# bbuchfink/diamond

Hardware: AMD Instinct MI355X
Metric: GCUPS + aligned queries/s, blastp --fast, 10000 queries vs 1000000-seq DB (seed stage + banded SW extension) (higher is better)
Workload: dtype int16

## Files before the change

### diamond_amd/csrc/api.hip

```cpp
#include <hip/hip_runtime.h>
#include <algorithm>
#include <atomic>
#include <chrono>
#include <time.h>
#include <cstdio>
#include <cstdlib>
#include <cstring>
#include <mutex>
#include <thread>
#include <numeric>
#include <unordered_map>
#include <string>
#include <vector>
#include "../../include/diamond_hip.h"
#include "swipe_core.h"
#include "swipe16_core.h"
#include "host_pool.h"
#include "swipe_kernels.h"
#include "ctx.h"
#include "score_matrices.h"

using namespace dmnd;

static thread_local std::string g_last_error;

int dmnd::fail(int code, const std::string& msg)
{
	g_last_error = msg;
	return code;
}

namespace {
std::mutex g_sync_mutex;
std::unordered_map<hipStream_t, hipEvent_t> g_sync_events;
}

static int sync_spin_us()
{
	return tuning().sync_spin_us;
}

hipError_t dmnd::wait_event(hipEvent_t ev, double* hint_us)
{
	if (spin_sync()) return hipEventSynchronize(ev);
	const int spin_us = sync_spin_us();
	auto t0 = std::chrono::steady_clock::now();
	const auto t_wait = t0;
	double fine_until_us = 0.0;
	auto finish = [&](hipError_t e) {
		if (hint_us) *hint_us = e == hipSuccess ? std::chrono::duration<double, std::micro>(std::chrono::steady_clock::now() - t_wait).count() : 0.0;
		return e;
	};
	if (hint_us && *hint_us > 2.0 * spin_us) {
		const hipError_t q = hipEventQuery(ev);
		if (q != hipErrorNotReady) return finish(q);
		const long ns = (long)(std::min(*hint_us, 50000.0) * 750.0);
		timespec ts{ 0, ns };
		nanosleep(&ts, nullptr);
		t0 = std::chrono::steady_clock::now();
		fine_until_us = 2.0 * std::min(*hint_us, 50000.0);
	}
	long sleep_ns = 20000;
	for (;;) {
		const hipError_t q = hipEventQuery(ev);
		if (q == hipSuccess) return finish(hipSuccess);
		if (q != hipErrorNotReady) return finish(q);
		if (std::chrono::duration_cast<std::chrono::microseconds>(std::chrono::steady_clock::now() - t0).count() < spin_us) continue;
		timespec ts{ 0, sleep_ns };
		nanosleep(&ts, nullptr);
		if (sleep_ns < 200000) sleep_ns += sleep_ns / 2;
		if (fine_until_us > 0.0 && sleep_ns > 50000 && std::chrono::duration<double, std::micro>(std::chrono::steady_clock::now() - t_wait).count() < fine_until_us) sleep_ns = 50000;
	}
}

hipError_t dmnd::sync_stream(hipStream_t s, double* hint_us)
{
	if (spin_sync()) return hipStreamSynchronize(s);
	hipEvent_t ev = nullptr;
	{
		std::lock_guard<std::mutex> g(g_sync_mutex);
		auto it = g_sync_events.find(s);
		if (it != g_sync_events.end()) ev = it->second;
		else {
			const hipError_t e = hipEventCreateWithFlags(&ev, hipEventBlockingSync | hipEventDisableTiming);
			if (e != hipSuccess) return e;
			g_sync_events[s] = ev;
		}
	}
	const hipError_t e = hipEventRecord(ev, s);
	if (e != hipSuccess) return e;
	return wait_event(ev, hint_us);
}

void dmnd::forget_stream(hipStream_t s)
{
	hipEvent_t ev = nullptr;
	{
		std::lock_guard<std::mutex> g(g_sync_mutex);
		auto it = g_sync_events.find(s);
// ... 421 lines not shown
	HIP_TRY(hipSetDevice(c->device));
	c->cbs_len = len;
	if (len == 0)
		return DMND_OK;
	c->cbs_generation = ~(uint64_t)0;
	if (int rc = c->cbs.ensure((size_t)len + 256)) return rc;
	HIP_TRY(hipMemcpyAsync(c->cbs.p, cbs, (size_t)len, hipMemcpyHostToDevice, c->stream));
	HIP_TRY(sync_stream(c->stream));
	return DMND_OK;
}

extern "C" int32_t dmnd_banded_cols(int32_t qlen, int32_t tlen, int32_t d_begin, int32_t d_end)
{
	const int32_t pos = std::max(d_end - 1, 0) - (d_end - 1);
	const int32_t j1 = std::min(qlen - 1 - d_begin, tlen - 1) + 1;
	return j1 - pos;
}

extern "C" double dmnd_evalue(const dmnd_ctx* c, int32_t raw_score, uint32_t query_len, uint32_t subject_len)
{
	return c ? c->evaluer.evalue(raw_score, query_len, subject_len) : 0.0;
}

extern "C" double dmnd_evalue_p(const dmnd_params* p, int32_t raw_score, uint32_t query_len, uint32_t subject_len)
{
	if (!p) return 0.0;
	Evaluer e;
	e.init(*p);
	return e.evalue(raw_score, query_len, subject_len);
}

extern "C" int dmnd_evalue_batch(const dmnd_params* p, const int32_t* raw_score, const int32_t* query_len, const int32_t* subject_len,
	int64_t n, double* out)
{
	if (!p || !raw_score || !query_len || !subject_len || !out || n < 0) return fail(DMND_E_ARG, "dmnd_evalue_batch: bad argument");
	Evaluer e;
	e.init(*p);
	for (int64_t i = 0; i < n; ++i)
		out[i] = e.evalue(raw_score[i], (unsigned)query_len[i], (unsigned)subject_len[i]);
	return DMND_OK;
}

extern "C" double dmnd_bitscore_p(const dmnd_params* p, double raw_score)
{
	if (!p) return 0.0;
	Evaluer e;
	e.init(*p);
	return e.bitscore(raw_score);
}

extern "C" double dmnd_bitscore(const dmnd_ctx* c, double raw_score)
{
	return c ? c->evaluer.bitscore(raw_score) : 0.0;
}

extern "C" int dmnd_last_kernel_ms(const dmnd_ctx* c, double* swipe_ms, double* traceback_ms)
{
	if (!c) return fail(DMND_E_ARG, "ctx is NULL");
	if (swipe_ms) *swipe_ms = c->swipe_ms;
	if (traceback_ms) *traceback_ms = c->traceback_ms;
	return DMND_OK;
}

namespace {

struct Bases {
	const int8_t* q; int64_t q_len;
	const int8_t* t; int64_t t_len;
	const int8_t* cbs; int64_t cbs_len;
	const int8_t* matrices = nullptr; int64_t n_matrices = 0;
};

enum { ADJ_CLASS = 1 << 20 };
struct Slot { int32_t item; int32_t P; int64_t steps; };
inline int band_p(const Slot& s) { return s.P & (ADJ_CLASS - 1); }
inline bool own_matrix(const Slot& s) { return (s.P & ADJ_CLASS) != 0; }

bool force_swipe32()
{
	static const bool v = [] { const char* e = std::getenv("DMND_SWIPE32"); return e && e[0] == '1'; }();
	return v;
}

}

int64_t dmnd::sweep_rows_min_items()
{
	if (force_swipe32()) return INT64_MAX;
	const char* e = std::getenv("DMND_SWEEP_ROWS");
	if (e && e[0] == '0') return INT64_MAX;
	if (e && e[0] == '1') return 0;
	return tuning().sweep_rows_min_items;
}

namespace {

inline int sweep_class(int band, int64_t steps, bool own, int kmode, bool rows)
{
	if (rows && !own && kmode <= K_TRACE && steps <= 2 * (int64_t)SW16_MAX_PAIRS) return band_class_rows(band);
	return band_class(band);
}

struct SweepLaunch { int64_t s0, s1; bool k16; int64_t pair_off; };

void plan_sweeps(const std::vector<Slot>& slots, int kmode, bool force32, std::vector<SweepLaunch>& launches, std::vector<int32_t>& pairs)
{
	const int64_t n = (int64_t)slots.size();
	launches.clear(); pairs.clear();
	for (int64_t s0 = 0; s0 < n;) {
		int64_t s1 = s0, max_steps = 0;
		while (s1 < n && slots[(size_t)s1].P == slots[(size_t)s0].P) { max_steps = std::max(max_steps, slots[(size_t)s1].steps); ++s1; }
		const bool k16 = !force32 && !force_swipe32() && kmode <= K_TRACE && !own_matrix(slots[(size_t)s0]) && sw16_class(slots[(size_t)s0].P) && max_steps <= 2 * (int64_t)SW16_MAX_PAIRS;
		launches.push_back(SweepLaunch{ s0, s1, k16, (int64_t)pairs.size() });
		if (k16) {
			const int64_t per = class_items_per_wave16(slots[(size_t)s0].P);
			for (int64_t s = s0; s < (s1 - s0 + per - 1) / per * per + s0; ++s)
				pairs.push_back(s < s1 ? slots[(size_t)s].item : -1);
		}
		s0 = s1;
	}
}

int issue_sweeps(dmnd_ctx* work, const Bases& b, const dmnd_dp_target* d_items, const std::vector<Slot>& slots, const std::vector<SweepLaunch>& launches,
	const int32_t* order_dev, const int64_t* trace_off_slot_dev, const int32_t* pairs_dev, const int64_t* trace_off_item_dev, uint8_t* trace_dev, int kmode)
{
	const bool trace = kmode == K_TRACE;
	for (const SweepLaunch& l : launches) {
		const int P = band_p(slots[(size_t)l.s0]);
		if (l.k16) {
			Swipe16Args a;
			a.qblock = b.q; a.tblock = b.t; a.cbs = b.cbs; a.matrix = work->matrix.as<int8_t>();
			a.items = d_items;
			a.pairs = pairs_dev + l.pair_off;
			a.trace_off = trace ? trace_off_item_dev : nullptr;
			a.trace = trace ? trace_dev : nullptr;
			a.ends = work->ends.as<SwipeEnd>();
			a.n_pairs = (l.s1 - l.s0 + class_items_per_wave16(P) - 1) / class_items_per_wave16(P);
			a.gap_open = work->params.gap_open; a.gap_extend = work->params.gap_extend;
			a.score_only = kmode == K_SCORE;
			HIP_TRY(launch_banded_swipe16(P, trace, a, work->stream));
		}
		else {
			SwipeArgs a;
			a.qblock = b.q; a.tblock = b.t; a.cbs = b.cbs; a.matrix = work->matrix.as<int8_t>(); a.matrices = b.matrices;
			a.items = d_items;
			a.order = order_dev + l.s0;
			a.trace_off = trace ? trace_off_slot_dev + l.s0 : nullptr;
			a.trace = trace ? trace_dev : nullptr;
			a.ends = work->ends.as<SwipeEnd>();
			a.n = l.s1 - l.s0;
			a.gap_open = work->params.gap_open; a.gap_extend = work->params.gap_extend;
			HIP_TRY(launch_banded_swipe(P, kmode, a, work->stream));
		}
	}
	return DMND_OK;
}

int launch_sweeps(dmnd_ctx* work, const Bases& b, const dmnd_dp_target* d_items, int64_t n_items_total, const std::vector<Slot>& slots,
	const int32_t* order_dev, const int64_t* trace_off_slot_dev, const std::vector<int64_t>* trace_off_slot, uint8_t* trace_dev, int kmode, bool force32)
{
	const int64_t n = (int64_t)slots.size();
	const bool trace = kmode == K_TRACE;
	std::vector<SweepLaunch> launches;
	std::vector<int32_t>& pairs = work->h_pairs;
	plan_sweeps(slots, kmode, force32, launches, pairs);
	if (!pairs.empty()) {
		if (int rc = work->pairs.ensure(pairs.size() * sizeof(int32_t))) return rc;
		HIP_TRY(hipMemcpyAsync(work->pairs.p, pairs.data(), pairs.size() * sizeof(int32_t), hipMemcpyHostToDevice, work->stream));
		if (trace) {
			std::vector<int64_t>& by_item = work->h_trace_off_item;
			by_item.assign((size_t)n_items_total, 0);
			for (int64_t s = 0; s < n; ++s) by_item[(size_t)slots[(size_t)s].item] = (*trace_off_slot)[(size_t)s];
			if (int rc = work->trace_off_item.ensure(by_item.size() * sizeof(int64_t))) return rc;
			HIP_TRY(hipMemcpyAsync(work->trace_off_item.p, by_item.data(), by_item.size() * sizeof(int64_t), hipMemcpyHostToDevice, work->stream));
		}
	}
	return issue_sweeps(work, b, d_items, slots, launches, order_dev, trace_off_slot_dev, work->pairs.as<int32_t>(), work->trace_off_item.as<int64_t>(), trace_dev, kmode);
}

void order_slots(std::vector<Slot>& v, std::vector<Slot>& tmp, std::vector<uint32_t>& count)
{
	if (v.size() < 2048) {
		std::sort(v.begin(), v.end(), [](const Slot& x, const Slot& y) { return x.P < y.P || (x.P == y.P && x.steps > y.steps); });
		return;
	}
	const int NB = 1024;
	count.assign((size_t)32 * NB + 1, 0);
	auto cls = [](const Slot& x) { return class_index(band_p(x)) + (own_matrix(x) ? 16 : 0); };
	auto bucket = [&](const Slot& x) { return (size_t)cls(x) * NB + (size_t)(NB - 1 - std::min<int64_t>(x.steps >> 4, NB - 1)); };
	for (const Slot& x : v) ++count[bucket(x) + 1];
	for (size_t i = 1; i < count.size(); ++i) count[i] += count[i - 1];
	tmp.resize(v.size());
	for (const Slot& x : v) tmp[count[bucket(x)]++] = x;
	v.swap(tmp);
}

int run_chunk(dmnd_ctx* c, const Bases& b, const dmnd_dp_target* items, int64_t n_items_total, const dmnd_dp_target* d_items, const std::vector<Slot>& slots,
	int kmode, dmnd_hsp* out, std::vector<uint8_t>* chunk_transcripts, std::vector<int64_t>* chunk_tr_off, bool force32 = false)
{
	const int64_t n = (int64_t)slots.size();
	if (n == 0) return DMND_OK;
	const bool trace = kmode == K_TRACE;
	std::vector<int32_t> order(n), p_of(n);
	std::vector<int64_t> trace_off(n + 1, 0), tr_off(n + 1, 0);
	for (int64_t s = 0; s < n; ++s) {
		order[s] = slots[s].item;
		p_of[s] = band_p(slots[s]);
		if (trace) {
			const dmnd_dp_target& it = items[slots[s].item];
			const Geom g = make_geom(it.query_len, it.target_len, it.d_begin, it.d_end);
			trace_off[s + 1] = trace_off[s] + trace_bytes(g, band_p(slots[s]));
// ... 159 lines not shown
		HIP_TRY(hipMemcpyAsync(c->items.p, rev.data(), m * sizeof(dmnd_dp_target), hipMemcpyHostToDevice, c->stream));
		const double ms_fwd = c->swipe_ms;
		if (int rc = run_chunk(c, b, rev.data(), m, c->items.as<dmnd_dp_target>(), rslots, K_STATS_BWD_REV, out, nullptr, nullptr)) return rc;
		(void)ms_fwd;
		HIP_TRY(copy_now(c->stream, ends.data(), c->ends.p, m * sizeof(SwipeEnd), hipMemcpyDeviceToHost));
		for (int64_t k = 0; k < m; ++k) {
			dmnd_hsp& h = out[src[k]];
			h.score = ends[k].score;
			h.q_begin = rev[k].query_len - (ends[k].end_i + 1);
			h.s_begin = rev[k].target_len - (ends[k].end_j + 1);
			h.mismatches = ends[k].stat_a;
			h.gap_openings = ends[k].stat_b;
			h.gaps = h.length - h.identities - h.mismatches;
		}
		return DMND_OK;
	}

	hsps.resize((size_t)n);
	int64_t used = 0;
	for (int64_t c0 = 0; c0 < n;) {
		int64_t c1 = c0;
		size_t bytes = 0;
		while (c1 < n) {
			const dmnd_dp_target& it = items[c1];
			const Geom g = make_geom(it.query_len, it.target_len, it.d_begin, it.d_end);
			const size_t need = (size_t)trace_bytes(g, band_p(slots[c1]));
			if (c1 > c0 && bytes + need > c->trace_arena_max) break;
			bytes += need;
			++c1;
		}
		std::vector<Slot> chunk(slots.begin() + c0, slots.begin() + c1);
		order_slots(chunk);
		std::vector<uint8_t> tr;
		std::vector<int64_t> tr_off;
		lap(0);
		if (int rc = run_chunk(c, b, items, n, c->items.as<dmnd_dp_target>(), chunk, K_TRACE, out, transcript ? &tr : nullptr, transcript ? &tr_off : nullptr)) return rc;
		lap(1);
		HIP_TRY(copy_now(c->stream, hsps.data() + c0, c->hsps.as<dmnd_hsp>() + c0, (size_t)(c1 - c0) * sizeof(dmnd_hsp), hipMemcpyDeviceToHost));
		std::vector<Slot> again;
		std::vector<uint8_t> tr2;
		std::vector<int64_t> tr_off2;
		for (const Slot& x : chunk) if (hsps[(size_t)x.item].transcript_len < 0) again.push_back(for_32_bits(x));
		if (!again.empty()) {
			std::sort(again.begin(), again.end(), by_class);
			if (int rc = run_chunk(c, b, items, n, c->items.as<dmnd_dp_target>(), again, K_TRACE, out, transcript ? &tr2 : nullptr, transcript ? &tr_off2 : nullptr, true)) return rc;
			for (const Slot& x : again)
				HIP_TRY(copy_now(c->stream, &hsps[(size_t)x.item], c->hsps.as<dmnd_hsp>() + x.item, sizeof(dmnd_hsp), hipMemcpyDeviceToHost));
		}
		if (!transcript) {
			for (int64_t i = c0; i < c1; ++i) { out[i] = hsps[i]; out[i].transcript_off = -1; }
			c0 = c1;
			continue;
		}
		std::vector<int64_t> slot_of((size_t)(c1 - c0)), slot2_of((size_t)(c1 - c0), -1);
		for (size_t s = 0; s < chunk.size(); ++s) slot_of[(size_t)(chunk[s].item - c0)] = (int64_t)s;
		for (size_t s = 0; s < again.size(); ++s) slot2_of[(size_t)(again[s].item - c0)] = (int64_t)s;
		for (int64_t i = c0; i < c1; ++i) {
			dmnd_hsp h = hsps[i];
			const int64_t s2 = slot2_of[(size_t)(i - c0)], s = slot_of[(size_t)(i - c0)];
			const uint8_t* src = s2 >= 0 ? tr2.data() + tr_off2[(size_t)s2] : tr.data() + tr_off[(size_t)s];
			const int64_t len = h.transcript_len + 1;
			if (used + len > transcript_cap)
				return fail(DMND_E_CAP, "dmnd_banded_swipe: transcript arena too small");
			std::memcpy(transcript + used, src, (size_t)len);
			h.transcript_off = used;
			used += len;
			out[i] = h;
		}
		c0 = c1;
	}
	if (transcript_used) *transcript_used = used;
	lap(2);
	return DMND_OK;
}

}

int dmnd_sweep_classes(dmnd_ctx* work, const dmnd_ctx* c, const dmnd_dp_target* d_items, const uint32_t* class_count, const uint32_t* class_max_steps, int n_classes,
	const int32_t* order_dev, const int64_t* off_slot_dev, const int32_t* pairs_dev, const int64_t* off_item_dev, uint8_t* trace_dev, SwipeEnd* ends_dev)
{
	if (!c || !work) return fail(DMND_E_ARG, "ctx is NULL");
	const int8_t* cbs = c->cbs_len > 0 ? c->cbs.as<int8_t>() : nullptr;
	int64_t s0 = 0, pair0 = 0;
	for (int k = 0; k < n_classes; ++k) {
		const int64_t count = class_count[k];
		if (count == 0) continue;
		const bool own = k >= 16;
		const int P = class_of_index(own ? k - 16 : k);
		const int64_t per = class_items_per_wave16(P), waves = (count + per - 1) / per;
		const bool k16 = !own && !force_swipe32() && sw16_class(P) && (int64_t)class_max_steps[k] <= 2 * (int64_t)SW16_MAX_PAIRS;
		if (row_class(P) && !k16) return fail(DMND_E_ARG, "dmnd_sweep_classes: a row class outside the 16-bit kernels");
		if (k16) {
			Swipe16Args a;
			a.qblock = c->block[DMND_QUERY].as<int8_t>(); a.tblock = c->block[DMND_TARGET].as<int8_t>(); a.cbs = cbs; a.matrix = c->matrix.as<int8_t>();
			a.items = d_items; a.pairs = pairs_dev + pair0; a.trace_off = trace_dev ? off_item_dev : nullptr; a.trace = trace_dev; a.ends = ends_dev;
			a.n_pairs = waves;
			a.gap_open = c->params.gap_open; a.gap_extend = c->params.gap_extend;
			a.score_only = trace_dev == nullptr;
			HIP_TRY(launch_banded_swipe16(P, trace_dev != nullptr, a, work->stream));
		}
		else {
			SwipeArgs a;
			a.qblock = c->block[DMND_QUERY].as<int8_t>(); a.tblock = c->block[DMND_TARGET].as<int8_t>(); a.cbs = cbs; a.matrix = c->matrix.as<int8_t>(); a.matrices = own ? work->adj_matrices.as<int8_t>() : nullptr;
			a.items = d_items; a.order = order_dev + s0; a.trace_off = trace_dev ? off_slot_dev + s0 : nullptr; a.trace = trace_dev; a.ends = ends_dev;
			a.n = count;
			a.gap_open = c->params.gap_open; a.gap_extend = c->params.gap_extend;
			HIP_TRY(launch_banded_swipe(P, trace_dev ? K_TRACE : K_SCORE, a, work->stream));
		}
		s0 += count; pair0 += waves * per;
	}
	return DMND_OK;
}

int dmnd_swipe_shared(dmnd_ctx* work, const dmnd_ctx* c, const dmnd_dp_target* items, int64_t n, int mode, uint32_t hsp_values,
	dmnd_hsp* out, uint8_t* transcript, int64_t transcript_cap, int64_t* transcript_used)
{
	if (!c || !work) return fail(DMND_E_ARG, "ctx is NULL");
	const Bases b{ c->block[DMND_QUERY].as<int8_t>(), c->block_len[DMND_QUERY], c->block[DMND_TARGET].as<int8_t>(), c->block_len[DMND_TARGET],
		c->cbs_len > 0 ? c->cbs.as<int8_t>() : nullptr, c->cbs_len, work->adj_matrices.as<int8_t>(), work->n_adj_matrices };
	if (work != c) {
		work->matrix.p = c->matrix.p; work->matrix.cap = c->matrix.cap; work->matrix.own = false;
		work->params = c->params; work->evaluer = c->evaluer;
	}
	return swipe_impl(work, b, items, n, mode, hsp_values, out, transcript, transcript_cap, transcript_used);
}

int dmnd_swipe_targets(dmnd_ctx* work, const dmnd_ctx* c, const int8_t* t, int64_t t_len, const dmnd_dp_target* items, int64_t n, int mode, uint32_t hsp_values,
	dmnd_hsp* out, uint8_t* transcript, int64_t transcript_cap, int64_t* transcript_used)
{
	if (!c || !work || !t) return fail(DMND_E_ARG, "ctx is NULL");
	const Bases b{ c->block[DMND_QUERY].as<int8_t>(), c->block_len[DMND_QUERY], t, t_len, c->cbs_len > 0 ? c->cbs.as<int8_t>() : nullptr, c->cbs_len,
		work->adj_matrices.as<int8_t>(), work->n_adj_matrices };
	if (work != c) {
		work->matrix.p = c->matrix.p; work->matrix.cap = c->matrix.cap; work->matrix.own = false;
		work->params = c->params; work->evaluer = c->evaluer;
	}
	return swipe_impl(work, b, items, n, mode, hsp_values, out, transcript, transcript_cap, transcript_used);
}

int dmnd_swipe_keep(dmnd_ctx* work, const dmnd_ctx* c, const dmnd_dp_target* items, int64_t n, int arena, dmnd_hsp* out, KeptTrace& kt)
{
	kt.arena = arena; kt.kept = false;
	if (!c || !work) return fail(DMND_E_ARG, "ctx is NULL");
	if (n == 0) return DMND_OK;
	const Bases b{ c->block[DMND_QUERY].as<int8_t>(), c->block_len[DMND_QUERY], c->block[DMND_TARGET].as<int8_t>(), c->block_len[DMND_TARGET],
		c->cbs_len > 0 ? c->cbs.as<int8_t>() : nullptr, c->cbs_len, work->adj_matrices.as<int8_t>(), work->n_adj_matrices };
	auto wall = [] { return std::chrono::duration<double, std::milli>(std::chrono::steady_clock::now().time_since_epoch()).count(); };
	const double t0 = wall();
	int64_t total = 0;
	bool usable = arena >= 0 && arena < 16 && n <= 0x7fffffff, in_range = true;
	const bool rows = n >= sweep_rows_min_items();
	static thread_local std::vector<Slot> slots, sort_tmp;
	static thread_local std::vector<uint32_t> sort_count;
	static thread_local std::vector<int64_t> rows_of;
	slots.resize((size_t)n); rows_of.resize((size_t)n);
	for (int64_t i = 0; i < n && usable; ++i) {
		const dmnd_dp_target& it = items[i];
		const int band = it.d_end - it.d_begin;
		if (band <= 0 || it.query_len <= 0 || it.target_len <= 0 || band_class(band) > 32) { usable = false; break; }
		in_range &= !(it.query_off < 0 || it.target_off < 0 || it.query_off + it.query_len > b.q_len || it.target_off + it.target_len > b.t_len
			|| (it.cbs_off >= 0 && (!b.cbs || it.cbs_off + it.query_len > b.cbs_len)) || (it.cbs_off <= -2 && (own_matrix_number(it.cbs_off) >= b.n_matrices || (own_matrix_biased(it.cbs_off) && (!b.cbs || it.query_off + it.query_len > b.cbs_len)))));
		const Geom g = make_geom(it.query_len, it.target_len, it.d_begin, it.d_end);
		const int P = sweep_class(band, n_steps(g), it.cbs_off <= -2, K_TRACE, rows);
		slots[(size_t)i] = Slot{ (int32_t)i, P | (it.cbs_off <= -2 ? (int)ADJ_CLASS : 0), n_steps(g) };
		rows_of[(size_t)i] = trace_bytes(g, P);
		total += rows_of[(size_t)i];
	}
	if (!usable || (size_t)total > work->trace_arena_max)
		return dmnd_swipe_shared(work, c, items, n, DMND_SWIPE_SCORE, 0, out, nullptr, 0, nullptr);
// ... 262 lines not shown
```

### diamond_amd/csrc/swipe16_kernels.hip

```cpp
#include <hip/hip_runtime.h>
#include <stdint.h>
#include <type_traits>
#include <utility>
#include "swipe16_core.h"
#include "swipe_kernels.h"

namespace dmnd {

__device__ __forceinline__ uint32_t shr1_z(uint32_t v) { return (uint32_t)__builtin_amdgcn_update_dpp(0, (int)v, 0x138, 0xf, 0xf, true); }
__device__ __forceinline__ uint32_t shl1_z(uint32_t v) { return (uint32_t)__builtin_amdgcn_update_dpp(0, (int)v, 0x130, 0xf, 0xf, true); }
__device__ __forceinline__ uint32_t shr1_in(uint32_t edge, uint32_t v) { return (uint32_t)__builtin_amdgcn_update_dpp((int)edge, (int)v, 0x138, 0xf, 0xf, false); }
__device__ __forceinline__ uint32_t shl1_in(uint32_t edge, uint32_t v) { return (uint32_t)__builtin_amdgcn_update_dpp((int)edge, (int)v, 0x130, 0xf, 0xf, false); }

__device__ __forceinline__ uint32_t rshr1_z(uint32_t v) { return (uint32_t)__builtin_amdgcn_update_dpp(0, (int)v, 0x111, 0xf, 0xf, true); }
__device__ __forceinline__ uint32_t rshl1_z(uint32_t v) { return (uint32_t)__builtin_amdgcn_update_dpp(0, (int)v, 0x101, 0xf, 0xf, true); }
__device__ __forceinline__ uint32_t rshr1_in(uint32_t edge, uint32_t v) { return (uint32_t)__builtin_amdgcn_update_dpp((int)edge, (int)v, 0x111, 0xf, 0xf, false); }
__device__ __forceinline__ uint32_t rshl1_in(uint32_t edge, uint32_t v) { return (uint32_t)__builtin_amdgcn_update_dpp((int)edge, (int)v, 0x101, 0xf, 0xf, false); }

__device__ __forceinline__ int rfl(int x) { return __builtin_amdgcn_readfirstlane(x); }
__device__ __forceinline__ int64_t rfl64(int64_t x)
{
	const uint32_t lo = (uint32_t)rfl((int)(uint32_t)x), hi = (uint32_t)rfl((int)(uint32_t)((uint64_t)x >> 32));
	return (int64_t)(((uint64_t)hi << 32) | lo);
}

struct Item16 {
	Geom g;
	SeqView v;
	int pairs;
};

__device__ __forceinline__ Item16 load_item(const dmnd_dp_target* items, int idx, const int8_t* qblock, const int8_t* tblock, const int8_t* cbs)
{
	const dmnd_dp_target it = items[idx];
	Item16 r;
	r.g = make_geom(rfl(it.query_len), rfl(it.target_len), rfl(it.d_begin), rfl(it.d_end));
	const int64_t c = rfl64(it.cbs_off);
	r.v = SeqView{ qblock + rfl64(it.query_off), tblock + rfl64(it.target_off), c >= 0 ? cbs + c : nullptr, nullptr };
	r.pairs = sw16_pairs(r.g);
	return r;
}

__device__ __forceinline__ Item16 load_item_row(const dmnd_dp_target* items, int idx, const int8_t* qblock, const int8_t* tblock, const int8_t* cbs)
{
	const dmnd_dp_target it = items[idx];
	Item16 r;
	r.g = make_geom(it.query_len, it.target_len, it.d_begin, it.d_end);
	r.v = SeqView{ qblock + it.query_off, tblock + it.target_off, it.cbs_off >= 0 ? cbs + it.cbs_off : nullptr, nullptr };
	r.pairs = sw16_pairs(r.g);
	return r;
}

template<int... R, typename F>
__device__ __forceinline__ void unrolled(std::integer_sequence<int, R...>, F&& f) { (f(std::integral_constant<int, R>()), ...); }

enum { EDGE_CHUNK = 256 };

template<int P, bool TRACE, bool COORDS = true>
__global__ __launch_bounds__(WAVES_PER_BLOCK * 64)
void banded_swipe16_kernel(const int8_t* __restrict__ qblock, const int8_t* __restrict__ tblock, const int8_t* __restrict__ cbs,
	const int8_t* __restrict__ matrix, const dmnd_dp_target* __restrict__ items, const int32_t* __restrict__ pairs,
	const int64_t* __restrict__ trace_off, uint8_t* __restrict__ trace, SwipeEnd* __restrict__ ends, int64_t n_pairs, int gap_open, int gap_extend)
{
	__shared__ uint16_t table[32 * 32];
	__shared__ uint4 edges[WAVES_PER_BLOCK][EDGE_CHUNK];
	for (int x = threadIdx.x; x < 32 * 32; x += blockDim.x)
		table[x] = sw16_table_entry(matrix, x);
	__syncthreads();

	const int lane = threadIdx.x & 63, wave = rfl((int)(threadIdx.x >> 6));
	const int64_t slot = (int64_t)blockIdx.x * WAVES_PER_BLOCK + wave;
	if (slot >= n_pairs)
		return;
	const int idxA = rfl(pairs[2 * slot]), idxB_raw = rfl(pairs[2 * slot + 1]);
	const bool hasB = idxB_raw >= 0;
	const int idxB = hasB ? idxB_raw : idxA;
	const Item16 A = load_item(items, idxA, qblock, tblock, cbs), B = load_item(items, idxB, qblock, tblock, cbs);
	const pk16 go = pk_both(gap_open + gap_extend), ge = pk_both(gap_extend);
	const int nA = A.pairs, nB = hasB ? B.pairs : 0;

	Lane16<P> st;
	lane16_init(st, A.g, A.v, B.g, B.v, lane);
	constexpr int G = Sw16Group<P>::G;
	uint8_t *recA = nullptr, *recB = nullptr;
	if (TRACE) {
		recA = trace + rfl64(trace_off[idxA]) + lane * 16;
		recB = trace + rfl64(trace_off[idxB]) + lane * 16;
	}
	uint4* const my_edges = edges[wave];

	pk16 S0[P], S1[P];
	lane16_scores(st, table, S0, S1);
	Edge16 e = sw16_edge(A.g, A.v, B.g, B.v, P, 0);
	Trace16Group<P> acc;

	auto pair_step = [&](auto r, int t, int tc) {
		constexpr int R = decltype(r)::value;
		const uint4 nx = my_edges[t - tc];
		lane16_advance(st, shl1_in(e.qq, st.QQ[1]), shl1_in(e.cc, st.CC[1]), shr1_in(e.tt, st.TT[P - 1]));
		pk16 N0[P], N1[P];
		lane16_scores(st, table, N0, N1);
		const uint32_t revt = 0xffffu - (uint32_t)t;
		pk16 tb0[P], tb1[P];
		lane16_step<P, TRACE, 0, COORDS>(st, S0, shr1_z(st.F[2 * P - 1]), go, ge, revt, tb0);
		lane16_step<P, TRACE, 1, COORDS>(st, S1, shl1_z(st.E[0]), go, ge, revt, tb1);
		if (TRACE) acc.template put<R>(tb0, tb1);
#pragma unroll
		for (int p = 0; p < P; ++p) { S0[p] = N0[p]; S1[p] = N1[p]; }
		e.qq = nx.x; e.tt = nx.y; e.cc = nx.z;
		if (R % 2 == 1) __builtin_amdgcn_sched_barrier(0);
	};
	const int nMax = nA > nB ? nA : nB, T = (nMax + G - 1) / G * G;
	for (int tc = 0; tc < T; tc += EDGE_CHUNK) {
		__builtin_amdgcn_wave_barrier();
#pragma unroll
		for (int r = lane; r < EDGE_CHUNK; r += 64) {
			const Edge16 x = sw16_edge(A.g, A.v, B.g, B.v, P, tc + 1 + r);
			my_edges[r] = make_uint4(x.qq, x.tt, x.cc, 0u);
		}
		__builtin_amdgcn_fence(__ATOMIC_RELEASE, "wavefront");
		__builtin_amdgcn_wave_barrier();
		__builtin_amdgcn_fence(__ATOMIC_ACQUIRE, "wavefront");
		const int te = tc + EDGE_CHUNK < T ? tc + EDGE_CHUNK : T;
		for (int t = tc; t < te; t += G) {
			unrolled(std::make_integer_sequence<int, G>(), [&](auto r) { pair_step(r, t + decltype(r)::value, tc); });
			if (TRACE) {
				if (t < nA) *reinterpret_cast<uint4*>(recA) = make_uint4(acc.a[0], acc.a[1], acc.a[2], acc.a[3]);
				if (t < nB) *reinterpret_cast<uint4*>(recB) = make_uint4(acc.b[0], acc.b[1], acc.b[2], acc.b[3]);
				recA += 1024; recB += 1024;
			}
		}
	}

#pragma unroll
	for (int item = 0; item < 2; ++item) {
		if (item == 1 && !hasB) break;
		int bs, bi, bj;
		lane16_finish<P, COORDS>(st, item ? B.g : A.g, item == 1, lane, bs, bi, bj);
#pragma unroll
		for (int off = 32; off >= 1; off >>= 1) {
			const int os = __shfl_xor(bs, off), oi = __shfl_xor(bi, off), oj = __shfl_xor(bj, off);
			if (better_end(os, oj, oi, bs, bj, bi)) { bs = os; bi = oi; bj = oj; }
		}
		if (lane == 0) {
			SwipeEnd x;
			x.score = bs; x.end_i = bi; x.end_j = bj; x.stat_a = 0; x.stat_b = 0;
			x.pad[0] = bs >= SW16_MAX_SCORE ? 1 : 0;
			x.pad[1] = x.pad[2] = 0;
			ends[item ? idxB : idxA] = x;
		}
	}
}

enum { ROW_EDGE_CHUNK = 60 };

template<int P, bool TRACE, bool COORDS = true>
__global__ __launch_bounds__(WAVES_PER_BLOCK * 64)
void banded_swipe16_rows_kernel(const int8_t* __restrict__ qblock, const int8_t* __restrict__ tblock, const int8_t* __restrict__ cbs,
	const int8_t* __restrict__ matrix, const dmnd_dp_target* __restrict__ items, const int32_t* __restrict__ pairs,
	const int64_t* __restrict__ trace_off, uint8_t* __restrict__ trace, SwipeEnd* __restrict__ ends, int64_t n_waves, int gap_open, int gap_extend)
{
	__shared__ uint16_t table[32 * 32];
	__shared__ uint4 edges[WAVES_PER_BLOCK][4][ROW_EDGE_CHUNK + 1];
	for (int x = threadIdx.x; x < 32 * 32; x += blockDim.x)
		table[x] = sw16_table_entry(matrix, x);
	__syncthreads();

	const int lane = threadIdx.x & 63, wave = rfl((int)(threadIdx.x >> 6)), row = lane >> 4, rl = lane & 15;
	const int64_t slot = (int64_t)blockIdx.x * WAVES_PER_BLOCK + wave;
	if (slot >= n_waves)
		return;
	const int idx0 = rfl(pairs[8 * slot]);
	const int idxA_raw = pairs[8 * slot + 2 * row], idxB_raw = pairs[8 * slot + 2 * row + 1];
	const bool hasA = idxA_raw >= 0, hasB = idxB_raw >= 0;
	const int idxA = hasA ? idxA_raw : idx0, idxB = hasB ? idxB_raw : idxA;
	auto again = [](int idx) { asm volatile("" : "+v"(idx)); return idx; };
	const pk16 go = pk_both(gap_open + gap_extend), ge = pk_both(gap_extend);
	int nA, nB;
	Lane16<P> st;
	pk16 S0[P], S1[P];
	Edge16 e;
	{
		const Item16 A = load_item_row(items, idxA, qblock, tblock, cbs), B = load_item_row(items, idxB, qblock, tblock, cbs);
		nA = hasA ? A.pairs : 0; nB = hasB ? B.pairs : 0;
		lane16_init(st, A.g, A.v, B.g, B.v, rl);
		lane16_scores(st, table, S0, S1);
		e = sw16_edge(A.g, A.v, B.g, B.v, P, 0, 15);
	}
	constexpr int G = Sw16Group<P>::G;
	uint8_t *recA = nullptr, *recB = nullptr;
	if (TRACE) {
		recA = trace + trace_off[idxA] + rl * 16;
		recB = trace + trace_off[idxB] + rl * 16;
	}
	uint4* const my_edges = edges[wave][row];
	Trace16Group<P> acc;

	auto pair_step = [&](auto r, int t, int tc) {
		constexpr int R = decltype(r)::value;
		const uint4 nx = my_edges[t - tc];
		lane16_advance(st, rshl1_in(e.qq, st.QQ[1]), rshl1_in(e.cc, st.CC[1]), rshr1_in(e.tt, st.TT[P - 1]));
		pk16 N0[P], N1[P];
		lane16_scores(st, table, N0, N1);
		const uint32_t revt = 0xffffu - (uint32_t)t;
		pk16 tb0[P], tb1[P];
		lane16_step<P, TRACE, 0, COORDS>(st, S0, rshr1_z(st.F[2 * P - 1]), go, ge, revt, tb0);
		lane16_step<P, TRACE, 1, COORDS>(st, S1, rshl1_z(st.E[0]), go, ge, revt, tb1);
		if (TRACE) acc.template put<R>(tb0, tb1);
#pragma unroll
		for (int p = 0; p < P; ++p) { S0[p] = N0[p]; S1[p] = N1[p]; }
		e.qq = nx.x; e.tt = nx.y; e.cc = nx.z;
		__builtin_amdgcn_sched_barrier(0);
	};
	int nMax = nA > nB ? nA : nB;
	nMax = max(max(__builtin_amdgcn_readlane(nMax, 0), __builtin_amdgcn_readlane(nMax, 16)), max(__builtin_amdgcn_readlane(nMax, 32), __builtin_amdgcn_readlane(nMax, 48)));
	const int T = (nMax + G - 1) / G * G;
	for (int tc = 0; tc < T; tc += ROW_EDGE_CHUNK) {
		__builtin_amdgcn_wave_barrier();
		{
			const Item16 A = load_item_row(items, again(idxA), qblock, tblock, cbs), B = load_item_row(items, again(idxB), qblock, tblock, cbs);
			for (int r = rl; r < ROW_EDGE_CHUNK; r += 16) {
				const Edge16 x = sw16_edge(A.g, A.v, B.g, B.v, P, tc + 1 + r, 15);
				my_edges[r] = make_uint4(x.qq, x.tt, x.cc, 0u);
			}
		}
		__builtin_amdgcn_fence(__ATOMIC_RELEASE, "wavefront");
		__builtin_amdgcn_wave_barrier();
		__builtin_amdgcn_fence(__ATOMIC_ACQUIRE, "wavefront");
		const int te = tc + ROW_EDGE_CHUNK < T ? tc + ROW_EDGE_CHUNK : T;
		for (int t = tc; t < te; t += G) {
			unrolled(std::make_integer_sequence<int, G>(), [&](auto r) { pair_step(r, t + decltype(r)::value, tc); });
			if (TRACE) {
				if (t < nA) *reinterpret_cast<uint4*>(recA) = make_uint4(acc.a[0], acc.a[1], acc.a[2], acc.a[3]);
				if (t < nB) *reinterpret_cast<uint4*>(recB) = make_uint4(acc.b[0], acc.b[1], acc.b[2], acc.b[3]);
				recA += 256; recB += 256;
			}
		}
	}

#pragma unroll
	for (int item = 0; item < 2; ++item) {
		const dmnd_dp_target it = items[again(item ? idxB : idxA)];
		const Geom g = make_geom(it.query_len, it.target_len, it.d_begin, it.d_end);
		int bs, bi, bj;
		lane16_finish<P, COORDS>(st, g, item == 1, rl, bs, bi, bj);
#pragma unroll
		for (int off = 8; off >= 1; off >>= 1) {
			const int os = __shfl_xor(bs, off), oi = __shfl_xor(bi, off), oj = __shfl_xor(bj, off);
			if (better_end(os, oj, oi, bs, bj, bi)) { bs = os; bi = oi; bj = oj; }
		}
		if (rl == 0 && (item ? hasB : hasA)) {
			SwipeEnd x;
			x.score = bs; x.end_i = bi; x.end_j = bj; x.stat_a = 0; x.stat_b = 0;
			x.pad[0] = bs >= SW16_MAX_SCORE ? 1 : 0;
			x.pad[1] = x.pad[2] = 0;
			ends[item ? idxB : idxA] = x;
		}
	}
}

template<int P>
static hipError_t launch16_rows(bool trace, const Swipe16Args& a, hipStream_t stream)
{
	const unsigned blocks = (unsigned)((a.n_pairs + WAVES_PER_BLOCK - 1) / WAVES_PER_BLOCK);
	if (blocks == 0)
		return hipSuccess;
	const dim3 grid(blocks), block(WAVES_PER_BLOCK * 64);
	if (trace) hipLaunchKernelGGL((banded_swipe16_rows_kernel<P, true>), grid, block, 0, stream, a.qblock, a.tblock, a.cbs, a.matrix, a.items, a.pairs, a.trace_off, a.trace, a.ends, a.n_pairs, a.gap_open, a.gap_extend);
	else if (a.score_only) hipLaunchKernelGGL((banded_swipe16_rows_kernel<P, false, false>), grid, block, 0, stream, a.qblock, a.tblock, a.cbs, a.matrix, a.items, a.pairs, a.trace_off, a.trace, a.ends, a.n_pairs, a.gap_open, a.gap_extend);
	else hipLaunchKernelGGL((banded_swipe16_rows_kernel<P, false>), grid, block, 0, stream, a.qblock, a.tblock, a.cbs, a.matrix, a.items, a.pairs, a.trace_off, a.trace, a.ends, a.n_pairs, a.gap_open, a.gap_extend);
	return hipGetLastError();
}

template<int P>
static hipError_t launch16_p(bool trace, const Swipe16Args& a, hipStream_t stream)
{
	const unsigned blocks = (unsigned)((a.n_pairs + WAVES_PER_BLOCK - 1) / WAVES_PER_BLOCK);
	if (blocks == 0)
		return hipSuccess;
	const dim3 grid(blocks), block(WAVES_PER_BLOCK * 64);
	if (trace) hipLaunchKernelGGL((banded_swipe16_kernel<P, true>), grid, block, 0, stream, a.qblock, a.tblock, a.cbs, a.matrix, a.items, a.pairs, a.trace_off, a.trace, a.ends, a.n_pairs, a.gap_open, a.gap_extend);
	else if (a.score_only) hipLaunchKernelGGL((banded_swipe16_kernel<P, false, false>), grid, block, 0, stream, a.qblock, a.tblock, a.cbs, a.matrix, a.items, a.pairs, a.trace_off, a.trace, a.ends, a.n_pairs, a.gap_open, a.gap_extend);
	else hipLaunchKernelGGL((banded_swipe16_kernel<P, false>), grid, block, 0, stream, a.qblock, a.tblock, a.cbs, a.matrix, a.items, a.pairs, a.trace_off, a.trace, a.ends, a.n_pairs, a.gap_open, a.gap_extend);
	return hipGetLastError();
}

hipError_t launch_banded_swipe16(int P, bool trace, const Swipe16Args& a, hipStream_t stream)
{
	switch (P) {
	case 1: return launch16_p<1>(trace, a, stream);
	case 2: return launch16_p<2>(trace, a, stream);
	case 4: return launch16_p<4>(trace, a, stream);
	case 3: return launch16_rows<3>(trace, a, stream);
	case 5: return launch16_rows<5>(trace, a, stream);
	default: return hipErrorInvalidValue;
	}
}

}

namespace { __global__ void touch_swipe16_kernel() {} }
extern "C" hipError_t dmnd_touch_swipe16(hipStream_t st) { hipLaunchKernelGGL(touch_swipe16_kernel, dim3(1), dim3(64), 0, st); return hipGetLastError(); }
```

### diamond_amd/csrc/swipe_kernels.h

```cpp
#pragma once
#include <hip/hip_runtime.h>
#include <stdint.h>
#include "../../include/diamond_hip.h"

namespace dmnd {

enum { WAVES_PER_BLOCK = 4 };

struct SwipeEnd {
	int32_t score, end_i, end_j, stat_a, stat_b, pad[3];
};

__host__ __device__ inline int64_t own_matrix_number(int64_t cbs_off) { return (-2 - cbs_off) & (DMND_CBS_MATRIX_WITH_BIAS - 1); }
__host__ __device__ inline bool own_matrix_biased(int64_t cbs_off) { return cbs_off <= -2 && ((-2 - cbs_off) & DMND_CBS_MATRIX_WITH_BIAS) != 0; }

enum { K_SCORE = 0, K_COORDS = 1, K_TRACE = 2, K_STATS_FWD = 3, K_STATS_BWD_REV = 4 };

struct SwipeArgs {
	const int8_t* qblock;
	const int8_t* tblock;
	const int8_t* cbs;
	const int8_t* matrix;
	const int8_t* matrices;
	const dmnd_dp_target* items;
	const int32_t* order;
	const int64_t* trace_off;
	uint8_t* trace;
	SwipeEnd* ends;
	int64_t n;
	int32_t gap_open, gap_extend;
};

struct TracebackArgs {
	const int8_t* qblock;
	const int8_t* tblock;
	const int8_t* cbs;
	const int8_t* matrix;
	const int8_t* matrices;
	const dmnd_dp_target* items;
	const int32_t* order;
	const int32_t* p_of_slot;
	const int64_t* trace_off;
	const int64_t* transcript_off;
	const uint8_t* trace;
	uint8_t* transcript;
	const SwipeEnd* ends;
	dmnd_hsp* hsps;
	int32_t* status;
	int64_t n;
	int32_t gap_open, gap_extend;
	int32_t transcript_from_first = 0;
};

struct Swipe16Args {
	const int8_t* qblock;
	const int8_t* tblock;
	const int8_t* cbs;
	const int8_t* matrix;
	const dmnd_dp_target* items;
	const int32_t* pairs;
	const int64_t* trace_off;
	uint8_t* trace;
	SwipeEnd* ends;
	int64_t n_pairs;
	int32_t gap_open, gap_extend;
	bool score_only = false;
};

hipError_t launch_banded_swipe(int P, int mode, const SwipeArgs& a, hipStream_t stream);
hipError_t launch_banded_swipe16(int P, bool trace, const Swipe16Args& a, hipStream_t stream);
hipError_t launch_traceback(const TracebackArgs& a, hipStream_t stream);

}
```

### diamond_amd/csrc/tuning.h

```cpp
#pragma once
#include <algorithm>
#include <cstdlib>

namespace dmnd {

struct Tuning {
	bool spin_sync = false;
	int sync_spin_us = 150;
	int pool_spins = 600;
	int extend_team = 8;
	int extend_split = 1;
	int extend_runners = 1;
	int extend_sub_threads = 0;
	int sweep_rows_min_items = 1 << 17;
	int extend_resweep_below_pct = 40;
	bool no_stream_priority = false;
	int seed_slots_x8 = 0;
	int seed_readback_bytes = 1 << 20;
	int seed_slices_budget_mb = 3072;
	long long seed_slices_min_letters = 1 << 20;
	long long seed_slices_max_joined = 1 << 20;
	int seed_sort_cap = 1 << 16;
};

inline const Tuning& tuning()
{
	static const Tuning t = [] {
		Tuning x;
		auto num = [](const char* name, int fallback) { const char* e = std::getenv(name); return e ? std::atoi(e) : fallback; };
		{ const char* e = std::getenv("DMND_SPIN_SYNC"); x.spin_sync = e && e[0] == '1'; }
		x.sync_spin_us = std::max(0, num("DMND_SYNC_SPIN_US", x.sync_spin_us));
		x.pool_spins = std::max(0, num("DMND_POOL_SPINS", x.pool_spins));
		x.extend_team = std::max(1, num("DMND_EXTEND_TEAM", x.extend_team));
		x.extend_split = std::max(1, std::min(64, num("DMND_EXTEND_SPLIT", x.extend_split)));
		x.extend_runners = std::max(1, num("DMND_EXTEND_RUNNERS", x.extend_runners));
		x.extend_sub_threads = std::max(0, num("DMND_EXTEND_SUB_THREADS", x.extend_sub_threads));
		x.sweep_rows_min_items = std::max(0, num("DMND_SWEEP_ROWS_MIN", x.sweep_rows_min_items));
		x.extend_resweep_below_pct = std::max(0, std::min(100, num("DMND_EXTEND_RESWEEP_BELOW_PCT", x.extend_resweep_below_pct)));
		x.no_stream_priority = std::getenv("DMND_NO_STREAM_PRIORITY") != nullptr;
		if (std::getenv("DMND_SEED_SLOTS_X8")) x.seed_slots_x8 = std::min(64, std::max(8, num("DMND_SEED_SLOTS_X8", 0)));
		return x;
	}();
	return t;
}

}
```

Before: 253.5.

## Fuse 16-bit banded sweep classes into a single multi-class kernel launch

```diff
diff --git a/diamond_amd/csrc/api.hip b/diamond_amd/csrc/api.hip
--- a/diamond_amd/csrc/api.hip
+++ b/diamond_amd/csrc/api.hip
@@ -15,6 +15,7 @@
 #include "../../include/diamond_hip.h"
 #include "swipe_core.h"
 #include "swipe16_core.h"
+#include "swipe16_fused.h"
 #include "host_pool.h"
 #include "swipe_kernels.h"
 #include "ctx.h"
@@ -602,6 +603,13 @@
 	return v;
 }
 
+bool sweep_fused(int n_classes, bool with_rows, int64_t n_items)
+{
+	const char* e = std::getenv("DMND_SWEEP_FUSED");
+	if (n_classes < 2 || (e && e[0] == '0')) return false;
+	return (e && e[0] == '1') || with_rows || n_items <= tuning().sweep_fused_waves_max_items;
+}
+
 }
 
 int64_t dmnd::sweep_rows_min_items()
@@ -645,8 +653,31 @@
 	const int32_t* order_dev, const int64_t* trace_off_slot_dev, const int32_t* pairs_dev, const int64_t* trace_off_item_dev, uint8_t* trace_dev, int kmode)
 {
 	const bool trace = kmode == K_TRACE;
+	bool fused[FUSED_CLASSES] = { false, false, false, false };
+	{
+		int64_t f_waves[FUSED_CLASSES] = { 0, 0, 0, 0 }, f_pair0[FUSED_CLASSES] = { 0, 0, 0, 0 }, f_items = 0;
+		int n_fused = 0;
+		for (const SweepLaunch& l : launches) {
+			const int P = band_p(slots[(size_t)l.s0]), s = l.k16 ? fused_slot_of_class(P) : -1;
+			if (s < 0 || fused[s]) continue;
+			fused[s] = true; f_waves[s] = (l.s1 - l.s0 + class_items_per_wave16(P) - 1) / class_items_per_wave16(P); f_pair0[s] = l.pair_off; ++n_fused;
+			f_items += l.s1 - l.s0;
+		}
+		if (sweep_fused(n_fused, fused[2] || fused[3], f_items)) {
+			Swipe16Args a;
+			a.qblock = b.q; a.tblock = b.t; a.cbs = b.cbs; a.matrix = work->matrix.as<int8_t>();
+			a.items = d_items; a.pairs = pairs_dev; a.trace_off = trace ? trace_off_item_dev : nullptr; a.trace = trace ? trace_dev : nullptr;
+			a.ends = work->ends.as<SwipeEnd>(); a.n_pairs = 0;
+			a.gap_open = work->params.gap_open; a.gap_extend = work->params.gap_extend;
+			a.score_only = kmode == K_SCORE;
+			HIP_TRY(launch_banded_swipe16_fused(trace, a, f_waves, f_pair0, work->stream));
+		}
+		else
+			for (bool& f : fused) f = false;
+	}
 	for (const SweepLaunch& l : launches) {
 		const int P = band_p(slots[(size_t)l.s0]);
+		if (l.k16 && fused_slot_of_class(P) >= 0 && fused[fused_slot_of_class(P)]) continue;
 		if (l.k16) {
 			Swipe16Args a;
 			a.qblock = b.q; a.tblock = b.t; a.cbs = b.cbs; a.matrix = work->matrix.as<int8_t>();
@@ -972,9 +1003,38 @@
 	if (!c || !work) return fail(DMND_E_ARG, "ctx is NULL");
 	const int8_t* cbs = c->cbs_len > 0 ? c->cbs.as<int8_t>() : nullptr;
 	int64_t s0 = 0, pair0 = 0;
+	bool fused[FUSED_CLASSES] = { false, false, false, false };
+	if (!force_swipe32()) {
+		int64_t f_waves[FUSED_CLASSES] = { 0, 0, 0, 0 }, f_pair0[FUSED_CLASSES] = { 0, 0, 0, 0 }, p0 = 0, f_items = 0;
+		int n_fused = 0;
+		for (int k = 0; k < n_classes && k < 16; ++k) {
+			const int64_t count = class_count[k];
+			if (count == 0) continue;
+			const int P = class_of_index(k), s = fused_slot_of_class(P);
+			const int64_t per = class_items_per_wave16(P), waves = (count + per - 1) / per;
+			if (s >= 0 && (int64_t)class_max_steps[k] <= 2 * (int64_t)SW16_MAX_PAIRS) { fused[s] = true; f_waves[s] = waves; f_pair0[s] = p0; ++n_fused; f_items += count; }
+			p0 += waves * per;
+		}
+		if (sweep_fused(n_fused, fused[2] || fused[3], f_items)) {
+			Swipe16Args a;
+			a.qblock = c->block[DMND_QUERY].as<int8_t>(); a.tblock = c->block[DMND_TARGET].as<int8_t>(); a.cbs = cbs; a.matrix = c->matrix.as<int8_t>();
+			a.items = d_items; a.pairs = pairs_dev; a.trace_off = trace_dev ? off_item_dev : nullptr; a.trace = trace_dev; a.ends = ends_dev;
+			a.n_pairs = 0;
+			a.gap_open = c->params.gap_open; a.gap_extend = c->params.gap_extend;
+			a.score_only = trace_dev == nullptr;
+			HIP_TRY(launch_banded_swipe16_fused(trace_dev != nullptr, a, f_waves, f_pair0, work->stream));
+		}
+		else
+			for (bool& f : fused) f = false;
+	}
 	for (int k = 0; k < n_classes; ++k) {
 		const int64_t count = class_count[k];
 		if (count == 0) continue;
+		if (k < 16 && fused_slot_of_class(class_of_index(k)) >= 0 && fused[fused_slot_of_class(class_of_index(k))]) {
+			const int64_t per = class_items_per_wave16(class_of_index(k));
+			s0 += count; pair0 += (count + per - 1) / per * per;
+			continue;
+		}
 		const bool own = k >= 16;
 		const int P = class_of_index(own ? k - 16 : k);
 		const int64_t per = class_items_per_wave16(P), waves = (count + per - 1) / per;
diff --git a/diamond_amd/csrc/swipe16_fused.h b/diamond_amd/csrc/swipe16_fused.h
--- /dev/null
+++ b/diamond_amd/csrc/swipe16_fused.h
@@ -0,0 +1,50 @@
+#pragma once
+#include <stdint.h>
+
+#if defined(__HIPCC__)
+#define DMND_FUSED_HD __host__ __device__ inline
+#else
+#define DMND_FUSED_HD inline
+#endif
+
+namespace dmnd {
+
+enum { FUSED_CLASSES = 4 };
+
+DMND_FUSED_HD int fused_class_of_slot(int s) { return s == 0 ? 1 : s == 1 ? 2 : s == 2 ? 3 : 5; }
+DMND_FUSED_HD int fused_slot_of_class(int P) { return P == 1 ? 0 : P == 2 ? 1 : P == 3 ? 2 : P == 5 ? 3 : -1; }
+
+struct FusedMap {
+	uint32_t groups[FUSED_CLASSES];
+	uint32_t waves[FUSED_CLASSES];
+	int64_t pair0[FUSED_CLASSES];
+};
+
+struct FusedSlot { int slot; uint32_t index; };
+
+template<typename U>
+DMND_FUSED_HD FusedSlot fused_slot_in(const uint32_t* groups, U N, U x)
+{
+	for (int s = 0; s < FUSED_CLASSES - 1; ++s) {
+		const U n = (U)groups[s];
+		if (n == N) break;
+		if (n != 0) {
+			const U before = x * n / N;
+			if ((x + 1) * n / N > before) return FusedSlot{ s, (uint32_t)before };
+			x -= before;
+			N -= n;
+		}
+	}
+	int last = FUSED_CLASSES - 1;
+	while (last > 0 && groups[last] == 0) --last;
+	return FusedSlot{ last, (uint32_t)x };
+}
+
+DMND_FUSED_HD FusedSlot fused_slot(const uint32_t* groups, uint32_t b)
+{
+	uint64_t N = 0;
+	for (int s = 0; s < FUSED_CLASSES; ++s) N += groups[s];
+	return N <= 0xffffu ? fused_slot_in<uint32_t>(groups, (uint32_t)N, b) : fused_slot_in<uint64_t>(groups, N, (uint64_t)b);
+}
+
+}
diff --git a/diamond_amd/csrc/swipe16_kernels.hip b/diamond_amd/csrc/swipe16_kernels.hip
--- a/diamond_amd/csrc/swipe16_kernels.hip
+++ b/diamond_amd/csrc/swipe16_kernels.hip
@@ -3,6 +3,7 @@
 #include <type_traits>
 #include <utility>
 #include "swipe16_core.h"
+#include "swipe16_fused.h"
 #include "swipe_kernels.h"
 
 namespace dmnd {
@@ -56,22 +57,13 @@
 
 enum { EDGE_CHUNK = 256 };
 
-template<int P, bool TRACE, bool COORDS = true>
-__global__ __launch_bounds__(WAVES_PER_BLOCK * 64)
-void banded_swipe16_kernel(const int8_t* __restrict__ qblock, const int8_t* __restrict__ tblock, const int8_t* __restrict__ cbs,
-	const int8_t* __restrict__ matrix, const dmnd_dp_target* __restrict__ items, const int32_t* __restrict__ pairs,
-	const int64_t* __restrict__ trace_off, uint8_t* __restrict__ trace, SwipeEnd* __restrict__ ends, int64_t n_pairs, int gap_open, int gap_extend)
-{
-	__shared__ uint16_t table[32 * 32];
-	__shared__ uint4 edges[WAVES_PER_BLOCK][EDGE_CHUNK];
-	for (int x = threadIdx.x; x < 32 * 32; x += blockDim.x)
-		table[x] = sw16_table_entry(matrix, x);
-	__syncthreads();
-
-	const int lane = threadIdx.x & 63, wave = rfl((int)(threadIdx.x >> 6));
-	const int64_t slot = (int64_t)blockIdx.x * WAVES_PER_BLOCK + wave;
-	if (slot >= n_pairs)
-		return;
+template<int P, bool TRACE, bool COORDS>
+__device__ __forceinline__
+void swipe16_wave_body(const int8_t* __restrict__ qblock, const int8_t* __restrict__ tblock, const int8_t* __restrict__ cbs,
+	const dmnd_dp_target* __restrict__ items, const int32_t* __restrict__ pairs, const int64_t* __restrict__ trace_off, uint8_t* __restrict__ trace,
+	SwipeEnd* __restrict__ ends, int64_t slot, int gap_open, int gap_extend, const uint16_t* table, uint4* const my_edges)
+{
+	const int lane = threadIdx.x & 63;
 	const int idxA = rfl(pairs[2 * slot]), idxB_raw = rfl(pairs[2 * slot + 1]);
 	const bool hasB = idxB_raw >= 0;
 	const int idxB = hasB ? idxB_raw : idxA;
@@ -87,7 +79,6 @@
 		recA = trace + rfl64(trace_off[idxA]) + lane * 16;
 		recB = trace + rfl64(trace_off[idxB]) + lane * 16;
 	}
-	uint4* const my_edges = edges[wave];
 
 	pk16 S0[P], S1[P];
 	lane16_scores(st, table, S0, S1);
@@ -152,24 +143,40 @@
 	}
 }
 
-enum { ROW_EDGE_CHUNK = 60 };
-
-template<int P, bool TRACE, bool COORDS = true>
-__global__ __launch_bounds__(WAVES_PER_BLOCK * 64)
-void banded_swipe16_rows_kernel(const int8_t* __restrict__ qblock, const int8_t* __restrict__ tblock, const int8_t* __restrict__ cbs,
-	const int8_t* __restrict__ matrix, const dmnd_dp_target* __restrict__ items, const int32_t* __restrict__ pairs,
-	const int64_t* __restrict__ trace_off, uint8_t* __restrict__ trace, SwipeEnd* __restrict__ ends, int64_t n_waves, int gap_open, int gap_extend)
-{
-	__shared__ uint16_t table[32 * 32];
-	__shared__ uint4 edges[WAVES_PER_BLOCK][4][ROW_EDGE_CHUNK + 1];
+__device__ __forceinline__ void fill_table16(uint16_t* table, const int8_t* __restrict__ matrix)
+{
 	for (int x = threadIdx.x; x < 32 * 32; x += blockDim.x)
 		table[x] = sw16_table_entry(matrix, x);
 	__syncthreads();
-
-	const int lane = threadIdx.x & 63, wave = rfl((int)(threadIdx.x >> 6)), row = lane >> 4, rl = lane & 15;
+}
+
+template<int P, bool TRACE, bool COORDS = true>
+__global__ __launch_bounds__(WAVES_PER_BLOCK * 64)
+void banded_swipe16_kernel(const int8_t* __restrict__ qblock, const int8_t* __restrict__ tblock, const int8_t* __restrict__ cbs,
+	const int8_t* __restrict__ matrix, const dmnd_dp_target* __restrict__ items, const int32_t* __restrict__ pairs,
+	const int64_t* __restrict__ trace_off, uint8_t* __restrict__ trace, SwipeEnd* __restrict__ ends, int64_t n_pairs, int gap_open, int gap_extend)
+{
+	__shared__ uint16_t table[32 * 32];
+	__shared__ uint4 edges[WAVES_PER_BLOCK][EDGE_CHUNK];
+	fill_table16(table, matrix);
+	const int wave = rfl((int)(threadIdx.x >> 6));
 	const int64_t slot = (int64_t)blockIdx.x * WAVES_PER_BLOCK + wave;
-	if (slot >= n_waves)
+	if (slot >= n_pairs)
 		return;
+	swipe16_wave_body<P, TRACE, COORDS>(qblock, tblock, cbs, items, pairs, trace_off, trace, ends, slot, gap_open, gap_extend, table, edges[wave]);
+}
+
+enum { ROW_EDGE_CHUNK = 60 };
+
+enum { ROW_EDGE_RECORDS = 4 * (ROW_EDGE_CHUNK + 1) };
+
+template<int P, bool TRACE, bool COORDS>
+__device__ __forceinline__
+void swipe16_rows_body(const int8_t* __restrict__ qblock, const int8_t* __restrict__ tblock, const int8_t* __restrict__ cbs,
+	const dmnd_dp_target* __restrict__ items, const int32_t* __restrict__ pairs, const int64_t* __restrict__ trace_off, uint8_t* __restrict__ trace,
+	SwipeEnd* __restrict__ ends, int64_t slot, int gap_open, int gap_extend, const uint16_t* table, uint4* const wave_edges)
+{
+	const int lane = threadIdx.x & 63, row = lane >> 4, rl = lane & 15;
 	const int idx0 = rfl(pairs[8 * slot]);
 	const int idxA_raw = pairs[8 * slot + 2 * row], idxB_raw = pairs[8 * slot + 2 * row + 1];
 	const bool hasA = idxA_raw >= 0, hasB = idxB_raw >= 0;
@@ -193,7 +200,7 @@
 		recA = trace + trace_off[idxA] + rl * 16;
 		recB = trace + trace_off[idxB] + rl * 16;
 	}
-	uint4* const my_edges = edges[wave][row];
+	uint4* const my_edges = wave_edges + row * (ROW_EDGE_CHUNK + 1);
 	Trace16Group<P> acc;
 
 	auto pair_step = [&](auto r, int t, int tc) {
@@ -259,6 +266,83 @@
 	}
 }
 
+template<int P, bool TRACE, bool COORDS = true>
+__global__ __launch_bounds__(WAVES_PER_BLOCK * 64)
+void banded_swipe16_rows_kernel(const int8_t* __restrict__ qblock, const int8_t* __restrict__ tblock, const int8_t* __restrict__ cbs,
+	const int8_t* __restrict__ matrix, const dmnd_dp_target* __restrict__ items, const int32_t* __restrict__ pairs,
+	const int64_t* __restrict__ trace_off, uint8_t* __restrict__ trace, SwipeEnd* __restrict__ ends, int64_t n_waves, int gap_open, int gap_extend)
+{
+	__shared__ uint16_t table[32 * 32];
+	__shared__ uint4 edges[WAVES_PER_BLOCK][ROW_EDGE_RECORDS];
+	fill_table16(table, matrix);
+	const int wave = rfl((int)(threadIdx.x >> 6));
+	const int64_t slot = (int64_t)blockIdx.x * WAVES_PER_BLOCK + wave;
+	if (slot >= n_waves)
+		return;
+	swipe16_rows_body<P, TRACE, COORDS>(qblock, tblock, cbs, items, pairs, trace_off, trace, ends, slot, gap_open, gap_extend, table, edges[wave]);
+}
+
+template<bool TRACE, bool COORDS, bool ROWS>
+__global__ __launch_bounds__(WAVES_PER_BLOCK * 64) __attribute__((amdgpu_waves_per_eu(ROWS ? 1 : 7)))
+void banded_swipe16_fused_kernel(const int8_t* __restrict__ qblock, const int8_t* __restrict__ tblock, const int8_t* __restrict__ cbs,
+	const int8_t* __restrict__ matrix, const dmnd_dp_target* __restrict__ items, const int32_t* __restrict__ pairs,
+	const int64_t* __restrict__ trace_off, uint8_t* __restrict__ trace, SwipeEnd* __restrict__ ends, const FusedMap map, int gap_open, int gap_extend)
+{
+	static_assert(ROW_EDGE_RECORDS <= EDGE_CHUNK, "the row classes' edge records fit the wavefront classes'");
+	__shared__ uint16_t table[32 * 32];
+	__shared__ uint4 edges[WAVES_PER_BLOCK][EDGE_CHUNK];
+	fill_table16(table, matrix);
+	const int wave = rfl((int)(threadIdx.x >> 6));
+	const uint32_t groups[FUSED_CLASSES] = { map.groups[0], map.groups[1], map.groups[2], map.groups[3] };
+	const FusedSlot f = fused_slot(groups, blockIdx.x);
+	const int64_t slot = (int64_t)f.index * WAVES_PER_BLOCK + wave;
+	switch (rfl(f.slot)) {
+	case 0:
+		if (slot < map.waves[0])
+			swipe16_wave_body<1, TRACE, COORDS>(qblock, tblock, cbs, items, pairs + map.pair0[0], trace_off, trace, ends, slot, gap_open, gap_extend, table, edges[wave]);
+		break;
+	case 1:
+		if (slot < map.waves[1])
+			swipe16_wave_body<2, TRACE, COORDS>(qblock, tblock, cbs, items, pairs + map.pair0[1], trace_off, trace, ends, slot, gap_open, gap_extend, table, edges[wave]);
+		break;
+	case 2:
+		if (ROWS && slot < map.waves[2])
+			swipe16_rows_body<3, TRACE, COORDS>(qblock, tblock, cbs, items, pairs + map.pair0[2], trace_off, trace, ends, slot, gap_open, gap_extend, table, edges[wave]);
+		break;
+	default:
+		if (ROWS && slot < map.waves[3])
+			swipe16_rows_body<5, TRACE, COORDS>(qblock, tblock, cbs, items, pairs + map.pair0[3], trace_off, trace, ends, slot, gap_open, gap_extend, table, edges[wave]);
+		break;
+	}
+}
+
+template<bool ROWS>
+static hipError_t launch16_fused(bool trace, const Swipe16Args& a, const FusedMap& map, unsigned blocks, hipStream_t stream)
+{
+	const dim3 grid(blocks), block(WAVES_PER_BLOCK * 64);
+	if (trace) hipLaunchKernelGGL((banded_swipe16_fused_kernel<true, true, ROWS>), grid, block, 0, stream, a.qblock, a.tblock, a.cbs, a.matrix, a.items, a.pairs, a.trace_off, a.trace, a.ends, map, a.gap_open, a.gap_extend);
+	else if (a.score_only) hipLaunchKernelGGL((banded_swipe16_fused_kernel<false, false, ROWS>), grid, block, 0, stream, a.qblock, a.tblock, a.cbs, a.matrix, a.items, a.pairs, a.trace_off, a.trace, a.ends, map, a.gap_open, a.gap_extend);
+	else hipLaunchKernelGGL((banded_swipe16_fused_kernel<false, true, ROWS>), grid, block, 0, stream, a.qblock, a.tblock, a.cbs, a.matrix, a.items, a.pairs, a.trace_off, a.trace, a.ends, map, a.gap_open, a.gap_extend);
+	return hipGetLastError();
+}
+
+hipError_t launch_banded_swipe16_fused(bool trace, const Swipe16Args& a, const int64_t* waves, const int64_t* pair0, hipStream_t stream)
+{
+	FusedMap map;
+	uint64_t blocks = 0;
+	for (int s = 0; s < FUSED_CLASSES; ++s) {
+		if (waves[s] < 0 || waves[s] > 0xffffffffll) return hipErrorInvalidValue;
+		map.waves[s] = (uint32_t)waves[s];
+		map.groups[s] = (uint32_t)((waves[s] + WAVES_PER_BLOCK - 1) / WAVES_PER_BLOCK);
+		map.pair0[s] = pair0[s];
+		blocks += map.groups[s];
+	}
+	if (blocks == 0)
+		return hipSuccess;
+	if (blocks > 0x7fffffffull) return hipErrorInvalidValue;
+	return map.groups[2] + map.groups[3] > 0 ? launch16_fused<true>(trace, a, map, (unsigned)blocks, stream) : launch16_fused<false>(trace, a, map, (unsigned)blocks, stream);
+}
+
 template<int P>
 static hipError_t launch16_rows(bool trace, const Swipe16Args& a, hipStream_t stream)
 {
diff --git a/diamond_amd/csrc/swipe_kernels.h b/diamond_amd/csrc/swipe_kernels.h
--- a/diamond_amd/csrc/swipe_kernels.h
+++ b/diamond_amd/csrc/swipe_kernels.h
@@ -69,6 +69,7 @@
 
 hipError_t launch_banded_swipe(int P, int mode, const SwipeArgs& a, hipStream_t stream);
 hipError_t launch_banded_swipe16(int P, bool trace, const Swipe16Args& a, hipStream_t stream);
+hipError_t launch_banded_swipe16_fused(bool trace, const Swipe16Args& a, const int64_t* waves, const int64_t* pair0, hipStream_t stream);
 hipError_t launch_traceback(const TracebackArgs& a, hipStream_t stream);
 
 }
diff --git a/diamond_amd/csrc/tuning.h b/diamond_amd/csrc/tuning.h
--- a/diamond_amd/csrc/tuning.h
+++ b/diamond_amd/csrc/tuning.h
@@ -12,7 +12,8 @@
 	int extend_split = 1;
 	int extend_runners = 1;
 	int extend_sub_threads = 0;
-	int sweep_rows_min_items = 1 << 17;
+	int sweep_rows_min_items = 1 << 15;
+	int sweep_fused_waves_max_items = 20000;
 	int extend_resweep_below_pct = 40;
 	bool no_stream_priority = false;
 	int seed_slots_x8 = 0;
@@ -36,6 +37,7 @@
 		x.extend_runners = std::max(1, num("DMND_EXTEND_RUNNERS", x.extend_runners));
 		x.extend_sub_threads = std::max(0, num("DMND_EXTEND_SUB_THREADS", x.extend_sub_threads));
 		x.sweep_rows_min_items = std::max(0, num("DMND_SWEEP_ROWS_MIN", x.sweep_rows_min_items));
+		x.sweep_fused_waves_max_items = std::max(0, num("DMND_SWEEP_FUSED_WAVES_MAX", x.sweep_fused_waves_max_items));
 		x.extend_resweep_below_pct = std::max(0, std::min(100, num("DMND_EXTEND_RESWEEP_BELOW_PCT", x.extend_resweep_below_pct)));
 		x.no_stream_priority = std::getenv("DMND_NO_STREAM_PRIORITY") != nullptr;
 		if (std::getenv("DMND_SEED_SLOTS_X8")) x.seed_slots_x8 = std::min(64, std::max(8, num("DMND_SEED_SLOTS_X8", 0)));
```

New measurement: 253.4. Within noise of the previous version (-0.0%).
